# borglab/gtsfm

Measured on NVIDIA H100. Metric: image_pairs_per_sec, higher is better.
Workload: dtype f32

## Files before the change

gtsfm_b200/_lib.py:

```python
from __future__ import annotations

import ctypes as C
from pathlib import Path
from typing import Optional

import numpy as np

LIB_PATH = Path(__file__).resolve().parent / "libgtsfm_b200.so"

_lib: Optional[C.CDLL] = None


class B200Error(RuntimeError):
    pass


class LightGlueParams(C.Structure):
    _fields_ = [("depth_confidence", C.c_double), ("width_confidence", C.c_double), ("filter_threshold", C.c_double),
                ("prune_min_kpts", C.c_int), ("fp16_attention", C.c_int)]


class LightGluePair(C.Structure):
    _fields_ = [("kp0", C.c_void_p), ("desc0", C.c_void_p), ("n0", C.c_int), ("kp1", C.c_void_p), ("desc1", C.c_void_p), ("n1", C.c_int),
                ("out_matches", C.c_void_p), ("out_scores", C.c_void_p), ("out_k", C.c_int), ("out_stop_layer", C.c_int),
# ... 80 lines not shown
                ("mask_count", C.c_int), ("votes", C.c_int * 4), ("winner", C.c_int), ("pose_cands", C.c_double * 21)]


class LmedsParams(C.Structure):
    _fields_ = [("confidence", C.c_double * 2)]


class LmedsTrace(C.Structure):
    _fields_ = [("cap", C.c_int), ("idx", C.c_void_p), ("nsol", C.c_void_p), ("models", C.c_void_p), ("medians", C.c_void_p),
                ("niters", C.c_int), ("drawn", C.c_int), ("slot", C.c_int), ("min_median", C.c_float), ("sigma", C.c_double),
                ("thr", C.c_float), ("count", C.c_int)]


_vp, _i, _f, _sz = C.c_void_p, C.c_int, C.c_float, C.c_size_t
_ip = C.POINTER(C.c_int)

SIGNATURES = {
    "b2_version": (_i, []),
    "b2_create": (_i, [_i, C.POINTER(_vp)]),
    "b2_destroy": (None, [_vp]),
    "b2_last_error": (C.c_char_p, [_vp]),
    "b2_launch_count": (C.c_uint64, [_vp]),
    "b2_h2d_bytes": (C.c_uint64, [_vp]),
    "b2_set_option": (C.c_int, [_vp, C.c_char_p, C.c_int64]),
    "b2_profile_start": (_i, [_vp, C.c_char_p]),
    "b2_profile_stop": (_i, [_vp, C.POINTER(C.c_double), C.POINTER(C.c_uint64), C.POINTER(C.c_double)]),
    "b2_debug_fetch": (C.c_int64, [_vp, C.c_char_p, _vp, C.c_int64]),
    "b2_debug_linear_host": (_i, [_vp, C.POINTER(LinearLaunch), C.POINTER(LinearProblem), _i]),
    "b2_debug_gemm_segments_host": (_i, [_vp, _vp, _vp, _vp, _i, _i, _i, _i, _vp, _vp, _i, _vp, _vp]),
    "b2_debug_attention_host": (_i, [_vp, _i, _ip, _ip, _i, _f, _i, _vp, _vp, _vp, _vp]),
    "b2_debug_superglue_assign_host": (_i, [_vp, _i, _i, _vp, _i, _i, _f, _i, _f, _vp, _vp, _vp, _vp, _vp, _vp, _vp, _ip, _ip]),
    "b2_debug_lightglue_assign_host": (_i, [_vp, _i, _i, _vp, _i, _i, _vp, _vp, _vp, _vp, _f, _vp, _vp, _vp, _vp, _vp, _vp, _vp, _ip,
                                            _ip]),
    "b2_superpoint_set_weights": (_i, [_vp, _vp, _sz]),
    "b2_superpoint_detect_dev": (_i, [_vp, _vp, _i, _i, _i, _sz, _f, _i, _i, _vp, _vp, _i, _ip, C.POINTER(C.c_uint64), _vp]),
    "b2_superpoint_describe_dev": (_i, [_vp, C.c_uint64, _vp, _i, _vp, _vp]),
    "b2_superpoint_extract_dev": (_i, [_vp, _vp, _i, _i, _i, _sz, _f, _i, _i, _i, _vp, _vp, _vp, _ip, _vp]),
    "b2_superpoint_extract_async_dev": (_i, [_vp, _vp, _i, _i, _i, _sz, _f, _i, _i, _i, _vp, _vp, _vp, _vp, _vp]),
    "b2_superpoint_finish_dev": (_i, [_vp, _vp]),
    "b2_topk_indices_dev": (_i, [_vp, _vp, _i, _i, _vp, _ip, _vp]),
    "b2_superpoint_detect_host": (_i, [_vp, _vp, _i, _i, _i, _f, _i, _i, _vp, _vp, _i, _ip, C.POINTER(C.c_uint64)]),
    "b2_superpoint_describe_host": (_i, [_vp, C.c_uint64, _vp, _i, _vp]),
    "b2_image_resize_dev": (_i, [_vp, _vp, _i, _i, _i, _sz, _vp, _i, _i, _vp]),
    "b2_lightglue_set_weights": (_i, [_vp, _vp, _sz]),
    "b2_lightglue_qkv_rows": (_i, [_vp]),
    "b2_lightglue_match_dev": (_i, [_vp, _vp, _vp, _i, _vp, _vp, _i, C.POINTER(LightGlueParams), _vp, _vp, _ip, _ip, _vp]),
    "b2_lightglue_match_host": (_i, [_vp, _vp, _vp, _i, _vp, _vp, _i, C.POINTER(LightGlueParams), _vp, _vp, _ip, _ip]),
    "b2_lightglue_match_batched_dev": (_i, [_vp, C.POINTER(LightGluePair), _i, C.POINTER(LightGlueParams), _vp]),
    "b2_lightglue_encoded_bytes": (_sz, [_i]),
    "b2_lightglue_encode_batched_dev": (_i, [_vp, C.POINTER(LightGlueImage), _i, C.POINTER(LightGlueParams), _vp]),
    "b2_superglue_set_weights": (_i, [_vp, _vp, _sz]),
    "b2_superglue_match_dev": (_i, [_vp, _vp, _vp, _vp, _i, _i, _i, _vp, _vp, _vp, _i, _i, _i, _i, _f, _vp, _vp, _ip, _vp]),
    "b2_superglue_match_host": (_i, [_vp, _vp, _vp, _vp, _i, _i, _i, _vp, _vp, _vp, _i, _i, _i, _i, _f, _vp, _vp, _ip]),
    "b2_netvlad_blob_floats": (_sz, []),
    "b2_netvlad_set_weights": (_i, [_vp, _vp, _sz]),
    "b2_netvlad_describe_dev": (_i, [_vp, _vp, _i, _i, _i, _vp, _vp]),
    "b2_netvlad_describe_host": (_i, [_vp, _vp, _i, _i, _i, _vp]),
    "b2_megaloc_blob_floats": (_sz, []),
    "b2_megaloc_set_weights": (_i, [_vp, _vp, _sz]),
    "b2_megaloc_describe_dev": (_i, [_vp, _vp, _i, _i, _i, _vp, _vp]),
    "b2_megaloc_describe_host": (_i, [_vp, _vp, _i, _i, _i, _vp]),
    "b2_megaloc_describe_u8_dev": (_i, [_vp, _vp, _i, _i, _i, _sz, _vp, _vp]),
    "b2_megaloc_resize_u8_dev": (_i, [_vp, _vp, _i, _i, _i, _sz, _vp, _vp]),
    "b2_similarity_pairs_host": (_i, [_vp, _vp, _i, _i, _i, _f, _vp, _vp]),
    "b2_ransac_essential_host": (_i, [_vp, _vp, _vp, _i, C.POINTER(RansacParams), _vp, _vp, _ip, _vp, _vp]),
    "b2_ransac_fundamental_host": (_i, [_vp, _vp, _vp, _i, C.POINTER(RansacParams), _vp, _vp, _ip]),
# ... 118 lines not shown
```

gtsfm_b200/csrc/lightglue.cu:

```cuda
#include <stdlib.h>

#include "common.cuh"
#include "linear.cuh"
#include "assign_ps.cuh"

namespace {
constexpr int LG_LAYERS = 9;
constexpr size_t LG_NFLOATS = 11851601;
constexpr int D = 256;

struct SelfW {
  float *wqkv, *bqkv, *wout, *bout, *w0, *b0, *lng, *lnb, *w3, *b3;
};
struct CrossW {
  float *wqv, *bqv, *wout, *bout, *w0, *b0, *lng, *lnb, *w3, *b3;
};
struct AssignW {
  float *wm, *bm, *wf, *bf;
};
struct ConfW {
  float *w, *b;
};
}

// ... 430 lines not shown
  if (j < n) {
    const float cm = cmax[j], cl = clog[j], l1 = l1g[j];
    for (int i0 = warp; i0 < m; i0 += LG_COL_WARPS * LG_COL_UNROLL) {
      float x[LG_COL_UNROLL], rm[LG_COL_UNROLL], rl[LG_COL_UNROLL], l0[LG_COL_UNROLL];
#pragma unroll
      for (int u = 0; u < LG_COL_UNROLL; ++u) {
        const int i = i0 + u * LG_COL_WARPS;
        const bool in = i < m;
        x[u] = in ? sim[(size_t)i * n + j] : 0.f;
        rm[u] = in ? rmax[i] : 0.f, rl[u] = in ? rlog[i] : 0.f, l0[u] = in ? l0g[i] : 0.f;
      }
#pragma unroll
      for (int u = 0; u < LG_COL_UNROLL; ++u) {
        const int i = i0 + u * LG_COL_WARPS;
        if (i < m) {
          const float sc = (((x[u] - rm[u]) - rl[u]) + ((x[u] - cm) - cl)) + (l0[u] + l1);
          if (sc > bv) bv = sc, bi = i;
        }
      }
    }
  }
  sv[warp][lane] = bv, si[warp][lane] = bi;
  __syncthreads();
  if (warp == 0 && j < n) {
    for (int w = 1; w < LG_COL_WARPS; ++w) {
      float ov = sv[w][lane];
      int oi = si[w][lane];
      if (ov > bv || (ov == bv && oi < bi)) bv = ov, bi = oi;
    }
    arg[j] = bi == 0x7fffffff ? 0 : bi;
  }
}

__global__ void __launch_bounds__(1024) k_lg_filter(const float* __restrict__ best0, const int* __restrict__ a0,
                                                     const int* __restrict__ a1, int m, float th, const int* __restrict__ ind0,
                                                     const int* __restrict__ ind1, long long* __restrict__ out,
                                                     float* __restrict__ outs, int* __restrict__ count) {
  __shared__ int wtot[32];
  __shared__ int carry;
  if (threadIdx.x == 0) carry = 0;
  __syncthreads();
  const int lane = threadIdx.x & 31, warp = threadIdx.x >> 5;
  for (int base = 0; base < m; base += 1024) {
    int i = base + threadIdx.x;
    bool valid = false;
    float ms = 0.f;
    int j = 0;
    if (i < m) {
      j = a0[i];
      bool mutual = a1[j] == i;
      ms = mutual ? expf(best0[i]) : 0.f;
      valid = mutual && ms > th;
    }
    unsigned vm = __ballot_sync(0xffffffffu, valid);
    if (lane == 0) wtot[warp] = __popc(vm);
    __syncthreads();
    if (warp == 0) {
      int w = wtot[lane], ws = w;
#pragma unroll
      for (int o = 1; o < 32; o <<= 1) {
        int u = __shfl_up_sync(0xffffffffu, ws, o);
        if (lane >= o) ws += u;
      }
      wtot[lane] = ws - w;
    }
    __syncthreads();
    int pos = carry + wtot[warp] + __popc(vm & ((1u << lane) - 1));
    if (valid) {
      out[2 * (size_t)pos] = ind0[i];
      out[2 * (size_t)pos + 1] = ind1[j];
      if (outs) outs[pos] = ms;
    }
    __syncthreads();
    if (threadIdx.x == 1023) carry = pos + (valid ? 1 : 0);
    __syncthreads();
  }
  if (threadIdx.x == 0) *count = carry;
}


struct LgStats {
  float *max, *log, *lsg;
};
struct LgAssign {
  const float* sim;
  int M, N;
  const float *z0, *z1;
  const int *ind0, *ind1;
  float thr;
  LgStats r, c;
  float* best0;
  int *arg0, *arg1;
  DevBuf *part, *bar;
  int* err_flag;
  long long* out_matches;
  float* out_scores;
  int* count;
};

static int lg_assign(b2_context* ctx, cudaStream_t st, const LgAssign& p, int path, int G, int* ran) {
  const float* sim = p.sim;
  const int M = p.M, N = p.N;
  const bool persistent = path == 0 ? assign_ps_fits(1, N) : path == 1;
  if (persistent && !assign_ps_fits(1, N)) return b2_fail(ctx, B2_ERR_ARG, "the persistent assignment kernel holds at most 6240 columns");
  if (ran) *ran = persistent ? 1 : 2;
  int rc;
  if (persistent) {
    B2_CUDA(ctx, p.part->ensure((size_t)G * 2 * N * sizeof(float)));
    B2_CUDA(ctx, p.bar->ensure(16));
    B2_CUDA(ctx, cudaMemsetAsync(p.bar->p, 0, 16, st));
    SinkArgs sa{};
    sa.Z = sim, sa.M = M, sa.N = N, sa.iters = 1, sa.u = p.r.max, sa.v = p.c.max;
    sa.rlog = p.r.log, sa.clog = p.c.log, sa.z0 = p.z0, sa.z1 = p.z1;
    sa.lsg0 = p.r.lsg, sa.lsg1 = p.c.lsg, sa.part = p.part->as<float>(), sa.bar = p.bar->as<unsigned>();
    sa.best0 = p.best0, sa.arg0 = p.arg0, sa.arg1 = p.arg1, sa.err_flag = p.err_flag;
    if ((rc = launch_assign_ps<1>(ctx, st, sa, G, "k_lg_assign"))) return rc;
  } else {
    B2_LAUNCH(ctx, k_lg_row_stats, cdiv(M, 8), 256, 0, st, sim, M, N, p.r.max, p.r.log, p.z0, p.r.lsg);
    B2_CHECK_LAUNCH(ctx);
    B2_LAUNCH(ctx, k_lg_col_stats, cdiv(N, 32), 1024, 0, st, sim, M, N, p.c.max, p.c.log, p.z1, p.c.lsg);
    B2_CHECK_LAUNCH(ctx);
    B2_LAUNCH(ctx, k_lg_row_argmax, cdiv(M, 8), 256, 0, st, sim, M, N, p.r.max, p.r.log, p.c.max, p.c.log, p.r.lsg, p.c.lsg, p.best0,
              p.arg0);
    B2_CHECK_LAUNCH(ctx);
    B2_LAUNCH(ctx, k_lg_col_argmax, cdiv(N, 32), 1024, 0, st, sim, M, N, p.r.max, p.r.log, p.c.max, p.c.log, p.r.lsg, p.c.lsg, p.arg1);
    B2_CHECK_LAUNCH(ctx);
  }
  B2_LAUNCH(ctx, k_lg_filter, 1, 1024, 0, st, p.best0, p.arg0, p.arg1, M, p.thr, p.ind0, p.ind1, p.out_matches, p.out_scores, p.count);
  B2_CHECK_LAUNCH(ctx);
  return B2_OK;
}

extern "C" int b2_lightglue_qkv_rows(int* out) {
  if (!out) return B2_ERR_ARG;
  for (int r = 0; r < 3 * D; ++r) out[r] = (r % D) * 3 + r / D;
  return B2_OK;
}

extern "C" int b2_lightglue_set_weights(b2_context* ctx, const float* blob, size_t n_floats) {
  if (!ctx || !blob) return B2_ERR_ARG;
  std::lock_guard<std::mutex> lk(ctx->mu);
  if (n_floats != LG_NFLOATS)
    return b2_fail(ctx, B2_ERR_ARG, "lightglue blob must hold 11851601 floats, got " + std::to_string(n_floats));
  cudaSetDevice(ctx->device);
  if (!ctx->lg) ctx->lg = new LightGlueState();
  LightGlueState* s = ctx->lg;
  std::vector<size_t> sizes;
  sizes.push_back(64);
  for (int i = 0; i < LG_LAYERS; ++i) {
    const size_t self_sz[] = {768 * 256, 768, 256 * 256, 256, 512 * 512, 512, 512, 512, 256 * 512, 256};
    const size_t cross_sz[] = {256 * 256, 256, 256 * 256, 256, 256 * 256, 256, 512 * 512, 512, 512, 512, 256 * 512, 256};
    for (size_t z : self_sz) sizes.push_back(z);
    for (size_t z : cross_sz) sizes.push_back(z);
  }
  for (int i = 0; i < LG_LAYERS; ++i) {
    const size_t asz[] = {256, 1, 256 * 256, 256};
    for (size_t z : asz) sizes.push_back(z);
  }
  for (int i = 0; i < LG_LAYERS - 1; ++i) sizes.push_back(256), sizes.push_back(1);
  constexpr int SELF_T = 10, LAYER_T = 22;
  std::vector<size_t> order(sizes.size());
// ... 354 lines not shown
    }
    act = lg_active_sides(s, np);
  }
  const TcWeights tw = lg_tw(s);
  int live[LG_MAX_PAIRS], nlive = 0;
  for (int p = 0; p < np; ++p) {
    pairs[p].out_stop_layer = s->pair[p].stop + 1;
    if (s->pair[p].n0 > 0 && s->pair[p].n1 > 0 && s->side[2 * p].n > 0 && s->side[2 * p + 1].n > 0) live[nlive++] = p;
  }
  if (nlive == 0) return B2_OK;
  for (int layer = 0; layer < LG_LAYERS; ++layer) {
    LinArgs g[LG_MAX_SIDES];
    JobList<HeadJob> hj{};
    int ns = 0, mx = 0;
    for (int li = 0; li < nlive; ++li) {
      if (s->pair[live[li]].stop != layer) continue;
      for (int side = 0; side < 2; ++side) {
        LgSide& sd = s->side[2 * live[li] + side];
        const float* x = sd.x[sd.cur].as<float>();
        LinArgs& a = g[ns];
        a.a1f = x, a.a1p = planes_of(sd.xs[sd.cur], (size_t)sd.cap * 256), a.lda1 = 256, a.K1 = 256, a.w = s->aw[layer].wf, a.ldb = 256;
        a.bias = s->aw[layer].bf, a.scale = 0.25f;
        a.cf = sd.md.as<float>(), a.ldc = 256, a.cp = planes_of(sd.md, (size_t)sd.cap * 256), a.ldch = 256, a.M = sd.n, a.N = 256;
        hj.j[ns] = {x, sd.n, s->aw[layer].wm, s->aw[layer].bm, nullptr, nullptr, sd.ls.as<float>()};
        mx = sd.n > mx ? sd.n : mx;
        ++ns;
      }
    }
    if (ns == 0) continue;
    if ((rc = run_linear(ctx, st, tw, g, ns, "lg_assign_proj"))) return rc;
    B2_LAUNCH(ctx, k_lg_rowheads, dim3(cdiv(mx, 8), ns), 256, 0, st, hj, (const float*)nullptr, (const float*)nullptr);
    B2_CHECK_LAUNCH(ctx);
  }
  {
    LinArgs gs[LG_MAX_PAIRS];
    for (int li = 0; li < nlive; ++li) {
      const int p = live[li];
      LgSide &a = s->side[2 * p], &b = s->side[2 * p + 1];
      B2_CUDA(ctx, s->sim[p].ensure((size_t)a.n * b.n * 4));
      LinArgs& g = gs[li];
      g.a1f = a.md.as<float>(), g.a1p = planes_of(a.md, (size_t)a.cap * 256), g.lda1 = 256, g.K1 = 256;
      g.bf = b.md.as<float>(), g.bp = planes_of(b.md, (size_t)b.cap * 256), g.ldb = 256;
      g.cf = s->sim[p].as<float>(), g.ldc = b.n, g.tc_want_f32 = true, g.M = a.n, g.N = b.n;
    }
    if ((rc = run_linear(ctx, st, tw, gs, nlive, "lg_assign_sim"))) return rc;
  }
  for (int li = 0; li < nlive; ++li) {
    const int p = live[li];
    LgSide &a = s->side[2 * p], &b = s->side[2 * p + 1];
    const LgAssign la{s->sim[p].as<float>(), a.n, b.n, a.ls.as<float>(), b.ls.as<float>(), a.ind[a.cur].as<int>(), b.ind[b.cur].as<int>(),
                      (float)prm->filter_threshold, {a.rmax.as<float>(), a.rlog.as<float>(), a.lsg.as<float>()},
                      {b.rmax.as<float>(), b.rlog.as<float>(), b.lsg.as<float>()}, a.amax.as<float>(), a.aidx.as<int>(), b.aidx.as<int>(),
                      &s->as_part, &s->as_bar, s->errflag.as<int>(), s->pair[p].out_matches, s->pair[p].out_scores,
                      counters + 4 * LG_MAX_PAIRS + p};
    if ((rc = lg_assign(ctx, st, la, 0, s->persist_ctas, nullptr))) return rc;
  }
  B2_CUDA(ctx, cudaMemcpyAsync(hread + 4 * LG_MAX_PAIRS, counters + 4 * LG_MAX_PAIRS, LG_MAX_PAIRS * sizeof(int), cudaMemcpyDeviceToHost, st));
  B2_CUDA(ctx, cudaMemcpyAsync(hread + 5 * LG_MAX_PAIRS, s->errflag.p, sizeof(int), cudaMemcpyDeviceToHost, st));
  B2_CUDA(ctx, cudaStreamSynchronize(st));
  if (s->use_tc && hread[5 * LG_MAX_PAIRS]) return b2_fail(ctx, B2_ERR_STATE, "wgmma pipeline timed out on an mbarrier (kernel bug)");
  for (int li = 0; li < nlive; ++li) pairs[live[li]].out_k = hread[4 * LG_MAX_PAIRS + live[li]];
  ctx->debug["lg_desc0"] = {s->side[0].x[s->side[0].cur].as<float>(), (int64_t)s->side[0].n * 256};
  ctx->debug["lg_desc1"] = {s->side[1].x[s->side[1].cur].as<float>(), (int64_t)s->side[1].n * 256};
  return B2_OK;
}

static int lg_match_pairs(b2_context* ctx, b2_lightglue_pair* pairs, int n_pairs, const b2_lightglue_params* prm, cudaStream_t st) {
  LightGlueState* s = ctx->lg;
  if (!s || !s->loaded) return b2_fail(ctx, B2_ERR_STATE, "lightglue weights not set");
  s->persist_ctas = ctx->sm_count - ctx->reserve_sms > 0 ? ctx->sm_count - ctx->reserve_sms : 1;
  const int bmax = ctx->lg_batch > 0 && ctx->lg_batch < LG_MAX_PAIRS ? ctx->lg_batch : LG_MAX_PAIRS;
  for (int p0 = 0; p0 < n_pairs; p0 += bmax) {
    const int np = n_pairs - p0 < bmax ? n_pairs - p0 : bmax;
    int rc = lg_match_batch(ctx, pairs + p0, np, prm, st);
    if (rc) return rc;
  }
  return B2_OK;
}

extern "C" int b2_lightglue_match_batched_dev(b2_context* ctx, b2_lightglue_pair* pairs, int n_pairs, const b2_lightglue_params* params,
                                              void* stream) {
  if (!ctx || !params || n_pairs < 0 || (n_pairs > 0 && !pairs)) return B2_ERR_ARG;
  for (int p = 0; p < n_pairs; ++p) {
    const b2_lightglue_pair& pr = pairs[p];
    if (pr.n0 < 0 || pr.n1 < 0) return B2_ERR_ARG;
    if (pr.n0 > 0 && pr.n1 > 0 && (!pr.kp0 || !pr.desc0 || !pr.kp1 || !pr.desc1 || !pr.out_matches)) return B2_ERR_ARG;
    if (((uintptr_t)pr.enc0 | (uintptr_t)pr.enc1) & 15) return B2_ERR_ARG;
  }
// ... 174 lines not shown
  B2_CUDA(ctx, cnt.ensure(16));
  std::vector<int> iota((size_t)(M > N ? M : N));
  for (size_t i = 0; i < iota.size(); ++i) iota[i] = (int)i;
  B2_CUDA(ctx, cudaMemcpyAsync(dsim.p, sim, (size_t)M * N * 4, cudaMemcpyHostToDevice, st));
  B2_CUDA(ctx, cudaMemcpyAsync(dz0.p, z0, (size_t)M * 4, cudaMemcpyHostToDevice, st));
  B2_CUDA(ctx, cudaMemcpyAsync(dz1.p, z1, (size_t)N * 4, cudaMemcpyHostToDevice, st));
  B2_CUDA(ctx, cudaMemcpyAsync(di0.p, ind0 ? ind0 : iota.data(), (size_t)M * 4, cudaMemcpyHostToDevice, st));
  B2_CUDA(ctx, cudaMemcpyAsync(di1.p, ind1 ? ind1 : iota.data(), (size_t)N * 4, cudaMemcpyHostToDevice, st));
  B2_CUDA(ctx, cudaMemsetAsync(err.p, 0, 16, st));
  const int G = ctas > 0 ? ctas : (ctx->sm_count - ctx->reserve_sms > 0 ? ctx->sm_count - ctx->reserve_sms : 1);
  float *r = rs.as<float>(), *c = cs.as<float>();
  const LgAssign p{dsim.as<float>(), M, N, dz0.as<float>(), dz1.as<float>(), di0.as<int>(), di1.as<int>(), threshold, {r, r + M, r + 2 * M},
                   {c, c + N, c + 2 * N}, dbest.as<float>(), da0.as<int>(), da1.as<int>(), &part, &bar, err.as<int>(),
                   out.as<long long>(), outs.as<float>(), cnt.as<int>()};
  const int rc = lg_assign(ctx, st, p, path, G, out_path);
  if (rc) return rc;
  int k = 0, e = 0;
  B2_CUDA(ctx, cudaMemcpyAsync(&k, cnt.p, 4, cudaMemcpyDeviceToHost, st));
  B2_CUDA(ctx, cudaMemcpyAsync(&e, err.p, 4, cudaMemcpyDeviceToHost, st));
  B2_CUDA(ctx, cudaMemcpyAsync(row_stats, rs.p, (size_t)3 * M * 4, cudaMemcpyDeviceToHost, st));
  B2_CUDA(ctx, cudaMemcpyAsync(col_stats, cs.p, (size_t)3 * N * 4, cudaMemcpyDeviceToHost, st));
  B2_CUDA(ctx, cudaMemcpyAsync(best0, dbest.p, (size_t)M * 4, cudaMemcpyDeviceToHost, st));
  B2_CUDA(ctx, cudaMemcpyAsync(arg0, da0.p, (size_t)M * 4, cudaMemcpyDeviceToHost, st));
  B2_CUDA(ctx, cudaMemcpyAsync(arg1, da1.p, (size_t)N * 4, cudaMemcpyDeviceToHost, st));
  B2_CUDA(ctx, cudaStreamSynchronize(st));
  if (k > 0) {
    B2_CUDA(ctx, cudaMemcpy(out_matches, out.p, (size_t)k * 16, cudaMemcpyDeviceToHost));
    B2_CUDA(ctx, cudaMemcpy(out_scores, outs.p, (size_t)k * 4, cudaMemcpyDeviceToHost));
  }
  *out_k = k;
  if (e) return b2_fail(ctx, B2_ERR_STATE, "the persistent assignment kernel timed out in its grid barrier (kernel bug)");
  return B2_OK;
}
```

include/gtsfm_b200.h:

```cpp
#ifndef GTSFM_B200_H
#define GTSFM_B200_H

#include <stddef.h>
#include <stdint.h>

#ifdef __cplusplus
extern "C" {
#endif

typedef struct b2_context b2_context;

int b2_version(void);
int b2_create(int device, b2_context** out);
void b2_destroy(b2_context* ctx);
const char* b2_last_error(const b2_context* ctx);
uint64_t b2_launch_count(const b2_context* ctx);
uint64_t b2_h2d_bytes(const b2_context* ctx);
int b2_set_option(b2_context* ctx, const char* name, int64_t value);
int b2_profile_start(b2_context* ctx, const char* kernel_prefix);
int b2_profile_stop(b2_context* ctx, double* total_ms, uint64_t* launches, double* work);
int64_t b2_debug_fetch(b2_context* ctx, const char* name, float* host_out, int64_t max_floats);

typedef struct b2_linear_problem {
  const float* a1; int lda1;
  const float* a2; int lda2;
  const float* b;  int ldb;
  const float* resid; int ldr;
  float* c; int ldc;
  uint16_t* c_hi; uint16_t* c_lo; int ldch;
  int m, n;
} b2_linear_problem;
typedef struct b2_linear_launch {
  int path;
  int k1, k2, per_problem_b;
  const float* bias;
  float scale;
  int relu, gelu, head_major, lo_unscaled;
  int resid_in_place;
} b2_linear_launch;
int b2_debug_linear_host(b2_context* ctx, const b2_linear_launch* launch, const b2_linear_problem* problems, int np);
int b2_debug_gemm_segments_host(b2_context* ctx, const float* A, const float* B, const float* bias, int M, int K, int nseg,
                                int rot_mask, const float* cs, const float* sn, int separate, uint16_t* out_hi,
                                uint16_t* out_lo);
int b2_debug_attention_host(b2_context* ctx, int np, const int* nq, const int* nk, int heads, float scale, int single,
                            const float* q, const float* k, const float* v, float* o);
int b2_debug_superglue_assign_host(b2_context* ctx, int path, int ctas, const float* Z, int M, int N, float alpha, int iters,
                                   float threshold, float* u, float* v, float* best0, int* arg0, int* arg1, uint32_t* out_matches,
                                   float* out_scores, int* out_k, int* out_path);
int b2_debug_lightglue_assign_host(b2_context* ctx, int path, int ctas, const float* sim, int M, int N, const float* z0,
                                   const float* z1, const int* ind0, const int* ind1, float threshold, float* row_stats,
                                   float* col_stats, float* best0, int* arg0, int* arg1, int64_t* out_matches, float* out_scores,
                                   int* out_k, int* out_path);

int b2_superpoint_set_weights(b2_context* ctx, const float* host_blob, size_t n_floats);

int b2_superpoint_detect_dev(b2_context* ctx, const uint8_t* image, int height, int width, int channels, size_t pitch,
                             float keypoint_threshold, int nms_radius, int border, float* out_xy, float* out_score,
                             int cap, int* out_n, uint64_t* out_map_token, void* stream);
int b2_superpoint_describe_dev(b2_context* ctx, uint64_t map_token, const float* xy, int n, float* out_desc, void* stream);
int b2_superpoint_extract_dev(b2_context* ctx, const uint8_t* image, int height, int width, int channels, size_t pitch,
                              float keypoint_threshold, int nms_radius, int border, int max_keypoints, float* out_xy,
                              float* out_score, float* out_desc, int* out_n, void* stream);
int b2_superpoint_extract_async_dev(b2_context* ctx, const uint8_t* image, int height, int width, int channels, size_t pitch,
                                    float threshold, int nms_radius, int border, int max_keypoints, float* out_xy,
                                    float* out_score, float* out_desc, int* out_n_pinned, void* stream);
int b2_superpoint_finish_dev(b2_context* ctx, void* stream);
int b2_topk_indices_dev(b2_context* ctx, const float* scores, int n, int k, int32_t* out_idx, int* out_k, void* stream);

int b2_superpoint_detect_host(b2_context* ctx, const uint8_t* image, int height, int width, int channels,
                              float keypoint_threshold, int nms_radius, int border, float* out_xy, float* out_score,
                              int cap, int* out_n, uint64_t* out_map_token);
int b2_superpoint_describe_host(b2_context* ctx, uint64_t map_token, const float* xy, int n, float* out_desc);

int b2_image_resize_dev(b2_context* ctx, const uint8_t* src, int height, int width, int channels, size_t pitch, uint8_t* dst,
                        int new_height, int new_width, void* stream);

int b2_lightglue_set_weights(b2_context* ctx, const float* host_blob, size_t n_floats);
int b2_lightglue_qkv_rows(int* out);

typedef struct b2_lightglue_params {
  double depth_confidence;
  double width_confidence;
  double filter_threshold;
  int prune_min_kpts;
  int fp16_attention;
// ... 246 lines not shown
```

profiles/lightglue_call_sites.py:

```python
#!/usr/bin/env python
from __future__ import annotations

import argparse
import json
import subprocess
import sys
from collections import deque
from pathlib import Path

import numpy as np

ROOT = Path(__file__).resolve().parent.parent
sys.path.insert(0, str(ROOT))

PEAK_FLOPS = 989e12
PEAK_BYTES = 3.35e12
LOOKAHEAD, NEW_FRAMES, THR_PX = 20, 2, 4.0

GEMM_SITES = ["lg_self_qkv", "lg_self_out", "lg_self_ffn0", "lg_self_ffn3", "lg_cross_qk", "lg_cross_v", "lg_cross_qv",
              "lg_cross_out", "lg_cross_ffn0", "lg_cross_ffn3", "lg_assign_proj", "lg_assign_sim"]
LG_KERNELS = ["k_lg_load_desc", "k_lg_posenc", "k_lg_enc_copy", "k_lg_split_rotary", "k_lg_ln_gelu", "k_lg_rowheads", "k_lg_prune_plan", "k_lg_gather",
              "k_lg_assign", "k_lg_row_stats", "k_lg_col_stats", "k_lg_row_argmax", "k_lg_col_argmax", "k_lg_filter"]
GEMM_SHAPE = {
    "lg_self_qkv": (768, 256), "lg_self_out": (256, 256), "lg_self_ffn0": (512, 512), "lg_self_ffn3": (256, 512),
    "lg_cross_qk": (256, 256), "lg_cross_v": (256, 256), "lg_cross_qv": (512, 256), "lg_cross_out": (256, 256),
    "lg_cross_ffn0": (512, 512), "lg_cross_ffn3": (256, 512), "lg_assign_proj": (256, 256)}
GEMM_ROW_BYTES = {
    "lg_self_out": 256 * 4 + 256 * 4, "lg_self_ffn0": 512 * 4 + 512 * 4, "lg_self_ffn3": 512 * 4 + 256 * 4 * 3,
    "lg_cross_qk": 256 * 4 + 256 * 4, "lg_cross_v": 256 * 4 + 256 * 4, "lg_cross_qv": 256 * 4 + 512 * 4,
    "lg_cross_out": 256 * 4 + 256 * 4, "lg_cross_ffn0": 512 * 4 + 512 * 4, "lg_cross_ffn3": 512 * 4 + 256 * 4 * 3,
    "lg_assign_proj": 256 * 4 + 256 * 4 * 2}


def qkv_row_bytes(fused: bool) -> int:
    return 256 * 4 + (768 * 4 + 2 * 64 * 4 if fused else 768 * 4)


LG_ROW_BYTES = {
    "k_lg_split_rotary": (768 * 4 + 64 * 4 + 768 * 4, 1.0),
    "k_lg_ln_gelu": (512 * 4 + 512 * 4, 2.0),
    "k_lg_rowheads": (256 * 4, 1.0 / 9 * 8),
}


def gpu_name() -> str:
    try:
        return subprocess.run(["nvidia-smi", "--query-gpu=name,power.limit,clocks.max.sm", "--format=csv,noheader"], capture_output=True,
                              text=True, timeout=30).stdout.strip()
    except Exception as e:
        return f"unknown ({e!r})"


def main():
    ap = argparse.ArgumentParser()
    ap.add_argument("--steps", type=int, default=2, help="steps per profiled row (their mean is reported)")
# ... 104 lines not shown
```

Baseline: 131.0.

## Fuse LightGlue assignment similarity GEMM with softmax stats and argmax on tensor cores

Adds a warp-specialized Hopper kernel that computes the descriptor similarity tile on the fly with TMA loads and wgmma (split hi/lo fp16 for near-fp32 accuracy). The kernel reduces row and column log-softmax statistics in one pass and the mutual argmax in a second pass, without writing the full similarity matrix. A finish kernel then merges the column partials and runs the mutual-nearest filter. This removes the separate sim GEMM and the multiple stats and argmax passes over an MxN matrix, at the cost of computing the GEMM twice and adding cross-CTA partial buffers and atomics. The old path is kept behind a branch.

```diff
diff --git a/gtsfm_b200/_lib.py b/gtsfm_b200/_lib.py
--- a/gtsfm_b200/_lib.py
+++ b/gtsfm_b200/_lib.py
@@ -136,6 +136,7 @@
     "b2_debug_superglue_assign_host": (_i, [_vp, _i, _i, _vp, _i, _i, _f, _i, _f, _vp, _vp, _vp, _vp, _vp, _vp, _vp, _ip, _ip]),
     "b2_debug_lightglue_assign_host": (_i, [_vp, _i, _i, _vp, _i, _i, _vp, _vp, _vp, _vp, _f, _vp, _vp, _vp, _vp, _vp, _vp, _vp, _ip,
                                             _ip]),
+    "b2_debug_lightglue_assign_desc_host": (_i, [_vp, _i, _vp, _vp, _vp, _vp, _vp, _vp, _f, _vp, _vp, _vp, _vp, _vp, _vp, _vp, _vp]),
     "b2_superpoint_set_weights": (_i, [_vp, _vp, _sz]),
     "b2_superpoint_detect_dev": (_i, [_vp, _vp, _i, _i, _i, _sz, _f, _i, _i, _vp, _vp, _i, _ip, C.POINTER(C.c_uint64), _vp]),
     "b2_superpoint_describe_dev": (_i, [_vp, C.c_uint64, _vp, _i, _vp, _vp]),
diff --git a/gtsfm_b200/csrc/lightglue.cu b/gtsfm_b200/csrc/lightglue.cu
--- a/gtsfm_b200/csrc/lightglue.cu
+++ b/gtsfm_b200/csrc/lightglue.cu
@@ -486,10 +486,11 @@
   }
 }
 
-__global__ void __launch_bounds__(1024) k_lg_filter(const float* __restrict__ best0, const int* __restrict__ a0,
-                                                     const int* __restrict__ a1, int m, float th, const int* __restrict__ ind0,
-                                                     const int* __restrict__ ind1, long long* __restrict__ out,
-                                                     float* __restrict__ outs, int* __restrict__ count) {
+struct LgStats {
+  float *max, *log, *lsg;
+};
+__device__ void lg_filter_block(const float* best0, const int* a0, const int* a1, int m, float th, const int* ind0, const int* ind1,
+                                long long* __restrict__ out, float* __restrict__ outs, int* __restrict__ count) {
   __shared__ int wtot[32];
   __shared__ int carry;
   if (threadIdx.x == 0) carry = 0;
@@ -531,11 +532,328 @@
   }
   if (threadIdx.x == 0) *count = carry;
 }
-
-
-struct LgStats {
-  float *max, *log, *lsg;
-};
+__global__ void __launch_bounds__(1024) k_lg_filter(const float* __restrict__ best0, const int* __restrict__ a0,
+                                                     const int* __restrict__ a1, int m, float th, const int* __restrict__ ind0,
+                                                     const int* __restrict__ ind1, long long* __restrict__ out,
+                                                     float* __restrict__ outs, int* __restrict__ count) {
+  lg_filter_block(best0, a0, a1, m, th, ind0, ind1, out, outs, count);
+}
+
+constexpr int LA_THREADS = 384;
+constexpr int LA_KC = D / GW_K;
+constexpr int LA_A_BYTES = LA_KC * 2 * GW_A_BYTES;
+constexpr int LA_B_BYTES = 2 * GW_B_BYTES;
+constexpr int LA_STAGES = 3;
+constexpr int LA_WPART = 2 * 8 * GW_N;
+constexpr size_t LA_SMEM = LA_A_BYTES + LA_STAGES * LA_B_BYTES + 1024  + 256 ;
+constexpr float LA_L2E = 1.4426950408889634f;
+
+struct LaPair {
+  int M, N, tiles_n, unit_end;
+  const float *z0, *z1;
+  LgStats r, c;
+  float* best0;
+  int *arg0, *arg1;
+  float2* part;
+  const int *ind0, *ind1;
+  long long* out;
+  float* outs;
+  int* count;
+};
+struct LaMaps {
+  CUtensorMap ah[LG_MAX_PAIRS], al[LG_MAX_PAIRS], bh[LG_MAX_PAIRS], bl[LG_MAX_PAIRS];
+};
+struct LaArgs {
+  LaPair p[LG_MAX_PAIRS];
+  int np, units;
+  float thr;
+  unsigned* cnt;
+  float2* wpart;
+  int* err_flag;
+};
+
+__device__ __forceinline__ void la_bar_consumers() { asm volatile("bar.sync 1, 256;" ::: "memory"); }
+__device__ __forceinline__ bool la_better(float v, int i, float bv, int bi) { return v > bv || (v == bv && i < bi); }
+__device__ __forceinline__ void la_merge(float& m, float& s, float m2, float s2) {
+  const float mx = fmaxf(m, m2);
+  if (mx == -INFINITY) {
+    s = 0.f;
+    return;
+  }
+  const float d = m - m2, e = tc::ex2(-fabsf(d) * LA_L2E);
+  s = d > 0.f ? fmaf(s2, e, s) : fmaf(s, e, s2);
+  m = mx;
+}
+
+template <int H, int B = H>
+__device__ __forceinline__ void la_scatter_stats(float* m, float* s, int lane) {
+  const bool up = lane & B;
+#pragma unroll
+  for (int k = 0; k < H; ++k) {
+    const float m2 = __shfl_xor_sync(0xffffffffu, up ? m[k] : m[k + H], B);
+    const float s2 = __shfl_xor_sync(0xffffffffu, up ? s[k] : s[k + H], B);
+    if (up) m[k] = m[k + H], s[k] = s[k + H];
+    la_merge(m[k], s[k], m2, s2);
+  }
+}
+template <int H, int B = H>
+__device__ __forceinline__ void la_scatter_best(float* v, int* i, int lane) {
+  const bool up = lane & B;
+#pragma unroll
+  for (int k = 0; k < H; ++k) {
+    const float v2 = __shfl_xor_sync(0xffffffffu, up ? v[k] : v[k + H], B);
+    const int i2 = __shfl_xor_sync(0xffffffffu, up ? i[k] : i[k + H], B);
+    if (up) v[k] = v[k + H], i[k] = i[k + H];
+    if (la_better(v2, i2, v[k], i[k])) v[k] = v2, i[k] = i2;
+  }
+}
+
+template <int PASS>
+__global__ void __launch_bounds__(LA_THREADS, 1) k_lg_assign_tc(const __grid_constant__ LaMaps maps, const __grid_constant__ LaArgs g) {
+  extern __shared__ unsigned char la_raw[];
+  __shared__ int la_last;
+  const uint32_t raw = tc::smem_u32(la_raw);
+  const uint32_t smem0 = (raw + 1023u) & ~1023u;
+  unsigned char* sm = la_raw + (smem0 - raw);
+  float2* cpart = g.wpart + (size_t)blockIdx.x * LA_WPART;
+  uint64_t* full = reinterpret_cast<uint64_t*>(sm + LA_A_BYTES + LA_STAGES * LA_B_BYTES);
+  uint64_t* empty = full + LA_STAGES;
+  uint64_t* afull = empty + LA_STAGES;
+  uint64_t* aempty = afull + 1;
+  const int t = threadIdx.x, warp = t >> 5, lane = t & 31;
+  if (t == 0) {
+    for (int s = 0; s < LA_STAGES; ++s) tc::mbar_init(&full[s], 1), tc::mbar_init(&empty[s], 8);
+    tc::mbar_init(afull, 1);
+    tc::mbar_init(aempty, 8);
+    tc::fence_mbar_init();
+  }
+  __syncthreads();
+  bool ok = true;
+  auto decode = [&](int u, int& z, int& m0) {
+    z = 0;
+    while (z + 1 < g.np && u >= g.p[z].unit_end) ++z;
+    m0 = (u - (z ? g.p[z - 1].unit_end : 0)) * GW_M;
+  };
+
+  if (warp >= 8) {
+    asm volatile("setmaxnreg.dec.sync.aligned.u32 40;\n" ::: "memory");
+    if (warp == 8 && lane == 0) {
+      int gk = 0, iu = 0;
+      for (int u = blockIdx.x; u < g.units; u += gridDim.x, ++iu) {
+        int z, m0;
+        decode(u, z, m0);
+        if (iu > 0) ok = tc::mbar_wait(aempty, (iu - 1) & 1) && ok;
+        tc::mbar_expect_tx(afull, LA_A_BYTES);
+        for (int kc = 0; kc < LA_KC; ++kc) {
+          tc::tma_load_2d(smem0 + kc * 2 * GW_A_BYTES, &maps.ah[z], afull, kc * GW_K, m0);
+          tc::tma_load_2d(smem0 + kc * 2 * GW_A_BYTES + GW_A_BYTES, &maps.al[z], afull, kc * GW_K, m0);
+        }
+        for (int tn = 0; tn < g.p[z].tiles_n; ++tn)
+          for (int kc = 0; kc < LA_KC; ++kc, ++gk) {
+            const int s = gk % LA_STAGES;
+            if (gk >= LA_STAGES) ok = tc::mbar_wait(&empty[s], ((gk / LA_STAGES) - 1) & 1) && ok;
+            const uint32_t sB = smem0 + LA_A_BYTES + s * LA_B_BYTES;
+            tc::mbar_expect_tx(&full[s], LA_B_BYTES);
+            tc::tma_load_2d(sB, &maps.bh[z], &full[s], kc * GW_K, tn * GW_N);
+            tc::tma_load_2d(sB + GW_B_BYTES, &maps.bl[z], &full[s], kc * GW_K, tn * GW_N);
+          }
+      }
+    }
+  } else {
+    asm volatile("setmaxnreg.inc.sync.aligned.u32 232;\n" ::: "memory");
+    const int wg = warp >> 2;
+    const int r0 = wg * 64 + (warp & 3) * 16 + (lane >> 2);
+    const int c2 = (lane & 3) * 2;
+    int gk = 0, iu = 0, it = 0;
+    for (int u = blockIdx.x; u < g.units; u += gridDim.x, ++iu) {
+      int z, m0;
+      decode(u, z, m0);
+      const LaPair& pr = g.p[z];
+      const int M = pr.M, N = pr.N, rb = m0 / GW_M;
+      float rv[2], rs[2];
+      int ri[2];
+#pragma unroll
+      for (int h = 0; h < 2; ++h) rv[h] = -INFINITY, rs[h] = 0.f, ri[h] = 0x7fffffff;
+      ok = tc::mbar_wait(afull, iu & 1) && ok;
+      for (int tn = 0; tn < pr.tiles_n; ++tn, ++it) {
+        const int n0 = tn * GW_N;
+        float acc0[64], acc1[64];
+        for (int kc = 0; kc < LA_KC; ++kc, ++gk) {
+          const int s = gk % LA_STAGES;
+          ok = tc::mbar_wait(&full[s], (gk / LA_STAGES) & 1) && ok;
+          const uint32_t aH = smem0 + kc * 2 * GW_A_BYTES + wg * (64 * 128), aL = aH + GW_A_BYTES;
+          const uint32_t bH = smem0 + LA_A_BYTES + s * LA_B_BYTES, bL = bH + GW_B_BYTES;
+          const uint64_t dAh = tc::wg_desc_sw128(aH), dAl = tc::wg_desc_sw128(aL), dBh = tc::wg_desc_sw128(bH), dBl = tc::wg_desc_sw128(bL);
+          tc::wg_fence();
+#pragma unroll
+          for (int ks = 0; ks < GW_K / 16; ++ks) {
+            const uint64_t adv = (uint64_t)(ks * 2);
+            const uint32_t first = (kc == 0 && ks == 0) ? 0u : 1u;
+            tc::wg_ss_n128(acc0, dAh + adv, dBh + adv, first);
+            tc::wg_ss_n128(acc1, dAh + adv, dBl + adv, first);
+            tc::wg_ss_n128(acc1, dAl + adv, dBh + adv, 1u);
+          }
+          tc::wg_commit();
+          if (kc > 0) {
+            tc::wg_wait<1>();
+            if (lane == 0) tc::mbar_arrive(&empty[(gk - 1) % LA_STAGES]);
+          }
+        }
+        tc::wg_wait<0>();
+        if (lane == 0) {
+          tc::mbar_arrive(&empty[(gk - 1) % LA_STAGES]);
+          if (tn == pr.tiles_n - 1) tc::mbar_arrive(aempty);
+        }
+        float* x = acc0;
+#pragma unroll
+        for (int i = 0; i < 64; ++i) x[i] = fmaf(acc1[i], tc::LO_INV, acc0[i]);
+        if (m0 + GW_M > M || n0 + GW_N > N) {
+#pragma unroll
+          for (int i = 0; i < 64; ++i) {
+            const int row = m0 + r0 + 8 * ((i >> 1) & 1), col = n0 + 8 * (i >> 2) + c2 + (i & 1);
+            if (row >= M || col >= N) x[i] = -INFINITY;
+          }
+        }
+        float2* cp = cpart + (it & 1) * 8 * GW_N + warp * GW_N;
+        if (PASS == 1) {
+#pragma unroll
+          for (int h = 0; h < 2; ++h) {
+            float tm = -INFINITY;
+#pragma unroll
+            for (int j = 0; j < 16; ++j) tm = fmaxf(tm, fmaxf(x[4 * j + 2 * h], x[4 * j + 2 * h + 1]));
+            tm = fmaxf(tm, __shfl_xor_sync(0xffffffffu, tm, 1));
+            tm = fmaxf(tm, __shfl_xor_sync(0xffffffffu, tm, 2));
+            const float nm = fmaxf(rv[h], tm);
+            if (nm != -INFINITY) {
+              float ts = 0.f;
+#pragma unroll
+              for (int j = 0; j < 16; ++j)
+                ts += tc::ex2((x[4 * j + 2 * h] - nm) * LA_L2E) + tc::ex2((x[4 * j + 2 * h + 1] - nm) * LA_L2E);
+              rs[h] = fmaf(rs[h], tc::ex2((rv[h] - nm) * LA_L2E), ts);
+              rv[h] = nm;
+            }
+          }
+          float cm[32], cs[32];
+#pragma unroll
+          for (int k = 0; k < 32; ++k) {
+            const float a = x[4 * (k >> 1) + (k & 1)], b = x[4 * (k >> 1) + 2 + (k & 1)];
+            cm[k] = fmaxf(a, b);
+            cs[k] = cm[k] == -INFINITY ? 0.f : 1.f + tc::ex2((fminf(a, b) - cm[k]) * LA_L2E);
+          }
+          la_scatter_stats<16>(cm, cs, lane), la_scatter_stats<8>(cm, cs, lane), la_scatter_stats<4>(cm, cs, lane);
+#pragma unroll
+          for (int q = 0; q < 4; ++q) {
+            const int k = 4 * (lane >> 2) + q;
+            __stcg(cp + 8 * (k >> 1) + c2 + (k & 1), make_float2(cm[q], cs[q]));
+          }
+        } else {
+          float ra[2], rl[2], r2[2];
+#pragma unroll
+          for (int h = 0; h < 2; ++h) {
+            const int row = m0 + r0 + 8 * h;
+            ra[h] = row < M ? __ldg(pr.r.max + row) : 0.f, rl[h] = row < M ? __ldg(pr.r.log + row) : 0.f;
+            r2[h] = row < M ? __ldg(pr.r.lsg + row) : 0.f;
+          }
+#pragma unroll
+          for (int hf = 0; hf < 4; ++hf) {
+            float cv[8];
+            int ci[8];
+#pragma unroll
+            for (int kk = 0; kk < 8; ++kk) {
+              const int k = 8 * hf + kk, j = k >> 1, e = k & 1, col = n0 + 8 * j + c2 + e;
+              const float ca = col < N ? __ldg(pr.c.max + col) : 0.f, cl = col < N ? __ldg(pr.c.log + col) : 0.f;
+              const float c3 = col < N ? __ldg(pr.c.lsg + col) : 0.f;
+              float sc[2];
+#pragma unroll
+              for (int h = 0; h < 2; ++h) {
+                const float v = x[4 * j + 2 * h + e];
+                sc[h] = (((v - ra[h]) - rl[h]) + ((v - ca) - cl)) + (r2[h] + c3);
+                if (sc[h] > rv[h]) rv[h] = sc[h], ri[h] = col;
+              }
+              cv[kk] = sc[0], ci[kk] = m0 + r0;
+              if (sc[1] > sc[0]) cv[kk] = sc[1], ci[kk] = m0 + r0 + 8;
+            }
+            la_scatter_best<4, 16>(cv, ci, lane), la_scatter_best<2, 8>(cv, ci, lane), la_scatter_best<1, 4>(cv, ci, lane);
+            const int k = 8 * hf + (lane >> 2);
+            __stcg(cp + 8 * (k >> 1) + c2 + (k & 1), make_float2(cv[0], __int_as_float(ci[0])));
+          }
+        }
+        la_bar_consumers();
+        if (t < GW_N && n0 + t < N) {
+          const float2* q = cpart + (it & 1) * 8 * GW_N + t;
+          float2 v8[8];
+#pragma unroll
+          for (int w = 0; w < 8; ++w) v8[w] = __ldcg(q + w * GW_N);
+          float2 r = v8[0];
+#pragma unroll
+          for (int w = 1; w < 8; ++w) {
+            const float2 v = v8[w];
+            if (PASS == 1) sk_merge(r.x, r.y, v.x, v.y);
+            else if (v.x > r.x) r = v;
+          }
+          pr.part[(size_t)rb * N + n0 + t] = r;
+        }
+      }
+#pragma unroll
+      for (int h = 0; h < 2; ++h) {
+        const int row = m0 + r0 + 8 * h;
+        if (PASS == 1) {
+          float s = rs[h];
+          s += __shfl_xor_sync(0xffffffffu, s, 1);
+          s += __shfl_xor_sync(0xffffffffu, s, 2);
+          if ((lane & 3) == 0 && row < M) pr.r.max[row] = rv[h], pr.r.log[row] = logf(s), pr.r.lsg[row] = sk_logsigmoid(pr.z0[row]);
+        } else {
+          float bv = rv[h];
+          int bi = ri[h];
+#pragma unroll
+          for (int o = 1; o < 4; o <<= 1) {
+            const float v2 = __shfl_xor_sync(0xffffffffu, bv, o);
+            const int i2 = __shfl_xor_sync(0xffffffffu, bi, o);
+            if (la_better(v2, i2, bv, bi)) bv = v2, bi = i2;
+          }
+          if ((lane & 3) == 0 && row < M) pr.best0[row] = bv, pr.arg0[row] = bi;
+        }
+      }
+      if (PASS == 1) {
+        __threadfence();
+        la_bar_consumers();
+        const int nrb = (M + GW_M - 1) / GW_M;
+        if (t == 0) la_last = atomicAdd(g.cnt + z, 1u) == (unsigned)(nrb - 1);
+        la_bar_consumers();
+        if (la_last) {
+          __threadfence();
+          for (int j = t; j < N; j += 256) {
+            float m = -INFINITY, s = 0.f;
+            for (int r = 0; r < nrb; ++r) {
+              const float2 v = __ldcg(pr.part + (size_t)r * N + j);
+              sk_merge(m, s, v.x, v.y);
+            }
+            pr.c.max[j] = m, pr.c.log[j] = logf(s), pr.c.lsg[j] = sk_logsigmoid(pr.z1[j]);
+          }
+        }
+      }
+    }
+  }
+  if (!ok && g.err_flag) *g.err_flag = 1;
+}
+
+__global__ void __launch_bounds__(1024) k_lg_assign_finish(const __grid_constant__ LaArgs g) {
+  const LaPair& pr = g.p[blockIdx.x];
+  const int nrb = (pr.M + GW_M - 1) / GW_M;
+  for (int j = threadIdx.x; j < pr.N; j += 1024) {
+    float m = -INFINITY;
+    int bi = 0x7fffffff;
+    for (int r = 0; r < nrb; ++r) {
+      const float2 v = pr.part[(size_t)r * pr.N + j];
+      if (v.x > m) m = v.x, bi = __float_as_int(v.y);
+    }
+    pr.arg1[j] = bi == 0x7fffffff ? 0 : bi;
+  }
+  __syncthreads();
+  lg_filter_block(pr.best0, pr.arg0, pr.arg1, pr.M, g.thr, pr.ind0, pr.ind1, pr.out, pr.outs, pr.count);
+}
+
+
 struct LgAssign {
   const float* sim;
   int M, N;
@@ -581,6 +899,59 @@
     B2_CHECK_LAUNCH(ctx);
   }
   B2_LAUNCH(ctx, k_lg_filter, 1, 1024, 0, st, p.best0, p.arg0, p.arg1, M, p.thr, p.ind0, p.ind1, p.out_matches, p.out_scores, p.count);
+  B2_CHECK_LAUNCH(ctx);
+  return B2_OK;
+}
+
+struct LgAssignTc {
+  Pl md0, md1;
+  int M, N;
+  const float *z0, *z1;
+  const int *ind0, *ind1;
+  LgStats r, c;
+  float* best0;
+  int *arg0, *arg1;
+  long long* out_matches;
+  float* out_scores;
+  int* count;
+};
+static int lg_assign_tc(b2_context* ctx, cudaStream_t st, const LgAssignTc* p, int np, float thr, int G, DevBuf& part, DevBuf& cnt,
+                        int* err_flag) {
+  if (np <= 0) return B2_OK;
+  if (np > LG_MAX_PAIRS) return b2_fail(ctx, B2_ERR_ARG, "lg_assign_tc: too many pairs in one launch");
+  if (!tma_encoder()) return b2_fail(ctx, B2_ERR_CUDA, "cuTensorMapEncodeTiled is not available (driver too old?)");
+  static thread_local LaMaps maps;
+  LaArgs a{};
+  size_t part_elems = 0;
+  bool ok = true;
+  double work = 0.0;
+  for (int i = 0; i < np; ++i) {
+    const LgAssignTc& x = p[i];
+    if (x.M <= 0 || x.N <= 0) return b2_fail(ctx, B2_ERR_ARG, "lg_assign_tc: empty pair");
+    ok = ok && tma_map_2d(&maps.ah[i], x.md0.hi, x.M, D, D, GW_M) && tma_map_2d(&maps.al[i], x.md0.lo, x.M, D, D, GW_M);
+    ok = ok && tma_map_2d(&maps.bh[i], x.md1.hi, x.N, D, D, GW_N) && tma_map_2d(&maps.bl[i], x.md1.lo, x.N, D, D, GW_N);
+    a.units += cdiv(x.M, GW_M);
+    a.p[i] = {x.M, x.N, cdiv(x.N, GW_N), a.units, x.z0, x.z1, x.r, x.c, x.best0, x.arg0, x.arg1, nullptr, x.ind0, x.ind1,
+              x.out_matches, x.out_scores, x.count};
+    part_elems += (size_t)cdiv(x.M, GW_M) * x.N;
+    work += 3.0 * 2.0 * x.M * x.N * D;
+  }
+  if (!ok) return b2_fail(ctx, B2_ERR_CUDA, "cuTensorMapEncodeTiled failed (assignment)");
+  const int grid = a.units < G ? a.units : G;
+  B2_CUDA(ctx, part.ensure((part_elems + (size_t)grid * LA_WPART) * sizeof(float2)));
+  B2_CUDA(ctx, cnt.ensure(LG_MAX_PAIRS * sizeof(unsigned)));
+  B2_CUDA(ctx, cudaMemsetAsync(cnt.p, 0, LG_MAX_PAIRS * sizeof(unsigned), st));
+  for (int i = 0, off = 0; i < np; off += cdiv(p[i].M, GW_M) * p[i].N, ++i) a.p[i].part = part.as<float2>() + off;
+  a.np = np, a.thr = thr, a.cnt = cnt.as<unsigned>(), a.wpart = part.as<float2>() + part_elems, a.err_flag = err_flag;
+  B2_CUDA(ctx, cudaFuncSetAttribute(k_lg_assign_tc<1>, cudaFuncAttributeMaxDynamicSharedMemorySize, (int)LA_SMEM));
+  B2_CUDA(ctx, cudaFuncSetAttribute(k_lg_assign_tc<2>, cudaFuncAttributeMaxDynamicSharedMemorySize, (int)LA_SMEM));
+  b2_prof_work(ctx, "k_lg_assign_stats", work);
+  B2_LAUNCH_NAMED(ctx, "k_lg_assign_stats", k_lg_assign_tc<1>, grid, LA_THREADS, LA_SMEM, st, maps, a);
+  B2_CHECK_LAUNCH(ctx);
+  b2_prof_work(ctx, "k_lg_assign_argmax", work);
+  B2_LAUNCH_NAMED(ctx, "k_lg_assign_argmax", k_lg_assign_tc<2>, grid, LA_THREADS, LA_SMEM, st, maps, a);
+  B2_CHECK_LAUNCH(ctx);
+  B2_LAUNCH(ctx, k_lg_assign_finish, np, 1024, 0, st, a);
   B2_CHECK_LAUNCH(ctx);
   return B2_OK;
 }
@@ -1001,7 +1372,19 @@
     B2_LAUNCH(ctx, k_lg_rowheads, dim3(cdiv(mx, 8), ns), 256, 0, st, hj, (const float*)nullptr, (const float*)nullptr);
     B2_CHECK_LAUNCH(ctx);
   }
-  {
+  if (s->use_tc) {
+    LgAssignTc la[LG_MAX_PAIRS];
+    for (int li = 0; li < nlive; ++li) {
+      const int p = live[li];
+      LgSide &a = s->side[2 * p], &b = s->side[2 * p + 1];
+      la[li] = {planes_of(a.md, (size_t)a.cap * 256), planes_of(b.md, (size_t)b.cap * 256), a.n, b.n, a.ls.as<float>(), b.ls.as<float>(),
+                a.ind[a.cur].as<int>(), b.ind[b.cur].as<int>(), {a.rmax.as<float>(), a.rlog.as<float>(), a.lsg.as<float>()},
+                {b.rmax.as<float>(), b.rlog.as<float>(), b.lsg.as<float>()}, a.amax.as<float>(), a.aidx.as<int>(), b.aidx.as<int>(),
+                s->pair[p].out_matches, s->pair[p].out_scores, counters + 4 * LG_MAX_PAIRS + p};
+    }
+    if ((rc = lg_assign_tc(ctx, st, la, nlive, (float)prm->filter_threshold, s->persist_ctas, s->as_part, s->as_bar, s->errflag.as<int>())))
+      return rc;
+  } else {
     LinArgs gs[LG_MAX_PAIRS];
     for (int li = 0; li < nlive; ++li) {
       const int p = live[li];
@@ -1013,16 +1396,16 @@
       g.cf = s->sim[p].as<float>(), g.ldc = b.n, g.tc_want_f32 = true, g.M = a.n, g.N = b.n;
     }
     if ((rc = run_linear(ctx, st, tw, gs, nlive, "lg_assign_sim"))) return rc;
-  }
-  for (int li = 0; li < nlive; ++li) {
-    const int p = live[li];
-    LgSide &a = s->side[2 * p], &b = s->side[2 * p + 1];
-    const LgAssign la{s->sim[p].as<float>(), a.n, b.n, a.ls.as<float>(), b.ls.as<float>(), a.ind[a.cur].as<int>(), b.ind[b.cur].as<int>(),
-                      (float)prm->filter_threshold, {a.rmax.as<float>(), a.rlog.as<float>(), a.lsg.as<float>()},
-                      {b.rmax.as<float>(), b.rlog.as<float>(), b.lsg.as<float>()}, a.amax.as<float>(), a.aidx.as<int>(), b.aidx.as<int>(),
-                      &s->as_part, &s->as_bar, s->errflag.as<int>(), s->pair[p].out_matches, s->pair[p].out_scores,
-                      counters + 4 * LG_MAX_PAIRS + p};
-    if ((rc = lg_assign(ctx, st, la, 0, s->persist_ctas, nullptr))) return rc;
+    for (int li = 0; li < nlive; ++li) {
+      const int p = live[li];
+      LgSide &a = s->side[2 * p], &b = s->side[2 * p + 1];
+      const LgAssign la{s->sim[p].as<float>(), a.n, b.n, a.ls.as<float>(), b.ls.as<float>(), a.ind[a.cur].as<int>(), b.ind[b.cur].as<int>(),
+                        (float)prm->filter_threshold, {a.rmax.as<float>(), a.rlog.as<float>(), a.lsg.as<float>()},
+                        {b.rmax.as<float>(), b.rlog.as<float>(), b.lsg.as<float>()}, a.amax.as<float>(), a.aidx.as<int>(), b.aidx.as<int>(),
+                        &s->as_part, &s->as_bar, s->errflag.as<int>(), s->pair[p].out_matches, s->pair[p].out_scores,
+                        counters + 4 * LG_MAX_PAIRS + p};
+      if ((rc = lg_assign(ctx, st, la, 0, s->persist_ctas, nullptr))) return rc;
+    }
   }
   B2_CUDA(ctx, cudaMemcpyAsync(hread + 4 * LG_MAX_PAIRS, counters + 4 * LG_MAX_PAIRS, LG_MAX_PAIRS * sizeof(int), cudaMemcpyDeviceToHost, st));
   B2_CUDA(ctx, cudaMemcpyAsync(hread + 5 * LG_MAX_PAIRS, s->errflag.p, sizeof(int), cudaMemcpyDeviceToHost, st));
@@ -1263,3 +1646,74 @@
   if (e) return b2_fail(ctx, B2_ERR_STATE, "the persistent assignment kernel timed out in its grid barrier (kernel bug)");
   return B2_OK;
 }
+
+extern "C" int b2_debug_lightglue_assign_desc_host(b2_context* ctx, int np, const int* M, const int* N, const float* md0, const float* md1,
+                                                   const float* z0, const float* z1, float threshold, float* row_stats, float* col_stats,
+                                                   float* best0, int* arg0, int* arg1, int64_t* out_matches, float* out_scores, int* out_k) {
+  if (!ctx || !M || !N || !md0 || !md1 || !z0 || !z1 || !row_stats || !col_stats || !best0 || !arg0 || !arg1 || !out_matches ||
+      !out_scores || !out_k || np <= 0 || np > LG_MAX_PAIRS)
+    return B2_ERR_ARG;
+  int SM = 0, SN = 0, mx = 0;
+  for (int i = 0; i < np; ++i) {
+    if (M[i] <= 0 || N[i] <= 0) return B2_ERR_ARG;
+    SM += M[i], SN += N[i];
+    mx = M[i] > mx ? M[i] : mx;
+    mx = N[i] > mx ? N[i] : mx;
+  }
+  std::lock_guard<std::mutex> lk(ctx->mu);
+  cudaSetDevice(ctx->device);
+  cudaStream_t st = ctx->stream;
+  DevBuf f0, f1, p0, p1, dz0, dz1, rs, cs, dbest, da0, da1, di, part, cnt, err, out, outs, dcnt;
+  B2_CUDA(ctx, f0.ensure((size_t)SM * D * 4));
+  B2_CUDA(ctx, f1.ensure((size_t)SN * D * 4));
+  B2_CUDA(ctx, p0.ensure((size_t)SM * D * 4));
+  B2_CUDA(ctx, p1.ensure((size_t)SN * D * 4));
+  B2_CUDA(ctx, dz0.ensure((size_t)SM * 4));
+  B2_CUDA(ctx, dz1.ensure((size_t)SN * 4));
+  B2_CUDA(ctx, rs.ensure((size_t)3 * SM * 4));
+  B2_CUDA(ctx, cs.ensure((size_t)3 * SN * 4));
+  B2_CUDA(ctx, dbest.ensure((size_t)SM * 4));
+  B2_CUDA(ctx, da0.ensure((size_t)SM * 4));
+  B2_CUDA(ctx, da1.ensure((size_t)SN * 4));
+  B2_CUDA(ctx, di.ensure((size_t)mx * 4));
+  B2_CUDA(ctx, err.ensure(16));
+  B2_CUDA(ctx, out.ensure((size_t)SM * 16));
+  B2_CUDA(ctx, outs.ensure((size_t)SM * 4));
+  B2_CUDA(ctx, dcnt.ensure((size_t)np * 4));
+  std::vector<int> iota((size_t)mx);
+  for (size_t i = 0; i < iota.size(); ++i) iota[i] = (int)i;
+  B2_CUDA(ctx, cudaMemcpyAsync(f0.p, md0, (size_t)SM * D * 4, cudaMemcpyHostToDevice, st));
+  B2_CUDA(ctx, cudaMemcpyAsync(f1.p, md1, (size_t)SN * D * 4, cudaMemcpyHostToDevice, st));
+  B2_CUDA(ctx, cudaMemcpyAsync(dz0.p, z0, (size_t)SM * 4, cudaMemcpyHostToDevice, st));
+  B2_CUDA(ctx, cudaMemcpyAsync(dz1.p, z1, (size_t)SN * 4, cudaMemcpyHostToDevice, st));
+  B2_CUDA(ctx, cudaMemcpyAsync(di.p, iota.data(), (size_t)mx * 4, cudaMemcpyHostToDevice, st));
+  B2_CUDA(ctx, cudaMemsetAsync(err.p, 0, 16, st));
+  const size_t n0 = (size_t)SM * D, n1 = (size_t)SN * D;
+  B2_LAUNCH(ctx, k_split_f32, (unsigned)((n0 + 255) / 256), 256, 0, st, f0.as<float>(), n0, p0.as<__half>(), p0.as<__half>() + n0);
+  B2_LAUNCH(ctx, k_split_f32, (unsigned)((n1 + 255) / 256), 256, 0, st, f1.as<float>(), n1, p1.as<__half>(), p1.as<__half>() + n1);
+  B2_CHECK_LAUNCH(ctx);
+  LgAssignTc la[LG_MAX_PAIRS];
+  float *r = rs.as<float>(), *c = cs.as<float>();
+  for (int i = 0, om = 0, on = 0; i < np; om += M[i], on += N[i], ++i)
+    la[i] = {{p0.as<__half>() + (size_t)om * D, p0.as<__half>() + n0 + (size_t)om * D},
+             {p1.as<__half>() + (size_t)on * D, p1.as<__half>() + n1 + (size_t)on * D},
+             M[i], N[i], dz0.as<float>() + om, dz1.as<float>() + on, di.as<int>(), di.as<int>(),
+             {r + om, r + SM + om, r + 2 * SM + om}, {c + on, c + SN + on, c + 2 * SN + on}, dbest.as<float>() + om, da0.as<int>() + om,
+             da1.as<int>() + on, out.as<long long>() + 2 * (size_t)om, outs.as<float>() + om, dcnt.as<int>() + i};
+  const int G = ctx->sm_count - ctx->reserve_sms > 0 ? ctx->sm_count - ctx->reserve_sms : 1;
+  int rc = lg_assign_tc(ctx, st, la, np, threshold, G, part, cnt, err.as<int>());
+  if (rc) return rc;
+  int e = 0;
+  B2_CUDA(ctx, cudaMemcpyAsync(out_k, dcnt.p, (size_t)np * 4, cudaMemcpyDeviceToHost, st));
+  B2_CUDA(ctx, cudaMemcpyAsync(&e, err.p, 4, cudaMemcpyDeviceToHost, st));
+  B2_CUDA(ctx, cudaMemcpyAsync(row_stats, rs.p, (size_t)3 * SM * 4, cudaMemcpyDeviceToHost, st));
+  B2_CUDA(ctx, cudaMemcpyAsync(col_stats, cs.p, (size_t)3 * SN * 4, cudaMemcpyDeviceToHost, st));
+  B2_CUDA(ctx, cudaMemcpyAsync(best0, dbest.p, (size_t)SM * 4, cudaMemcpyDeviceToHost, st));
+  B2_CUDA(ctx, cudaMemcpyAsync(arg0, da0.p, (size_t)SM * 4, cudaMemcpyDeviceToHost, st));
+  B2_CUDA(ctx, cudaMemcpyAsync(arg1, da1.p, (size_t)SN * 4, cudaMemcpyDeviceToHost, st));
+  B2_CUDA(ctx, cudaMemcpyAsync(out_matches, out.p, (size_t)SM * 16, cudaMemcpyDeviceToHost, st));
+  B2_CUDA(ctx, cudaMemcpyAsync(out_scores, outs.p, (size_t)SM * 4, cudaMemcpyDeviceToHost, st));
+  B2_CUDA(ctx, cudaStreamSynchronize(st));
+  if (e) return b2_fail(ctx, B2_ERR_STATE, "the fused assignment timed out on an mbarrier (kernel bug)");
+  return B2_OK;
+}
diff --git a/include/gtsfm_b200.h b/include/gtsfm_b200.h
--- a/include/gtsfm_b200.h
+++ b/include/gtsfm_b200.h
@@ -51,6 +51,9 @@
                                    const float* z1, const int* ind0, const int* ind1, float threshold, float* row_stats,
                                    float* col_stats, float* best0, int* arg0, int* arg1, int64_t* out_matches, float* out_scores,
                                    int* out_k, int* out_path);
+int b2_debug_lightglue_assign_desc_host(b2_context* ctx, int np, const int* M, const int* N, const float* md0, const float* md1,
+                                        const float* z0, const float* z1, float threshold, float* row_stats, float* col_stats,
+                                        float* best0, int* arg0, int* arg1, int64_t* out_matches, float* out_scores, int* out_k);
 
 int b2_superpoint_set_weights(b2_context* ctx, const float* host_blob, size_t n_floats);
 
diff --git a/profiles/lightglue_call_sites.py b/profiles/lightglue_call_sites.py
--- a/profiles/lightglue_call_sites.py
+++ b/profiles/lightglue_call_sites.py
@@ -20,7 +20,8 @@
 GEMM_SITES = ["lg_self_qkv", "lg_self_out", "lg_self_ffn0", "lg_self_ffn3", "lg_cross_qk", "lg_cross_v", "lg_cross_qv",
               "lg_cross_out", "lg_cross_ffn0", "lg_cross_ffn3", "lg_assign_proj", "lg_assign_sim"]
 LG_KERNELS = ["k_lg_load_desc", "k_lg_posenc", "k_lg_enc_copy", "k_lg_split_rotary", "k_lg_ln_gelu", "k_lg_rowheads", "k_lg_prune_plan", "k_lg_gather",
-              "k_lg_assign", "k_lg_row_stats", "k_lg_col_stats", "k_lg_row_argmax", "k_lg_col_argmax", "k_lg_filter"]
+              "k_lg_assign", "k_lg_row_stats", "k_lg_col_stats", "k_lg_row_argmax", "k_lg_col_argmax", "k_lg_filter",
+              "k_lg_assign_stats", "k_lg_assign_argmax", "k_lg_assign_finish"]
 GEMM_SHAPE = {
     "lg_self_qkv": (768, 256), "lg_self_out": (256, 256), "lg_self_ffn0": (512, 512), "lg_self_ffn3": (256, 512),
     "lg_cross_qk": (256, 256), "lg_cross_v": (256, 256), "lg_cross_qv": (512, 256), "lg_cross_out": (256, 256),
```

Result: faster. 133.0 (median of 6 runs) (+1.5%).
